# si220/Forest-SLAM

Measured on AMD Instinct MI355X. Metric: stereo frames/sec (extract+match+local-BA) at 600p, 1/8 MI355X; ATE RMSE, higher is better.
Workload: dtype mixed: u8/u16 integer (FAST, BRIEF, Hamming, SGM), f32 (ORB angle/Harris, back-projection), f64 (PnP, BA incl. its Schur GEMM on f64 MFMA); 1 GPU; stereo VO front end, configs[1]: 960x600, ORB nfeatures=1000, BF-Hamming xcheck (L+R), SGBM-3way 96 disp, back-projection, PnP-RANSAC, local BA K=10; width=960, height=600, nfeatures=1000, local_ba=window K=10 per frame, 10 LM iterations (fvo_ba_windows), parallelism=seq-per-gpu x1

## Files before the change

forest-slam_amd/csrc/ba.hip:

```cpp
#include <cfloat>
#include <type_traits>

#include "fvo_device.h"

namespace {

struct BaObs {
  int lm;
  short frame, oct;
  float u, v, ur;
};

struct BaCam {
  double fx, fy, cx, cy, b;
};

constexpr int kKMax = kBaMaxWindow;
constexpr int kBldL = 0, kBldO = kKMax, kBldTot = 2 * kKMax, kBldF = 2 * kKMax + 2, kBldInts = 3 * kKMax + 2;
constexpr int kBlock = 256;
constexpr int kLinParts = 12, kLinChunksPerPart = 8;
constexpr int kLinLPC64 = 64, kLinWavesDefault = 16;
static_assert(64 * kLinWavesDefault / (kLinLPC64 / 2) <= 64 && 64 * kLinWavesDefault / kLinLPC64 >= 16,
              "a landmark's lane group fits one wave and holds K observations");
constexpr int kLinWaves = kLinWavesDefault, kLinBlock = 64 * kLinWaves;
constexpr int kLinProd = kLinWaves / 2, kLinCons = kLinWaves - kLinProd;
constexpr int kLinMaxTiles = (36 + kLinCons - 1) / kLinCons;
constexpr int kLinTiles64 = (10 + kLinCons - 1) / kLinCons;
static_assert(kLinLPC64 / 2 <= 32 && (3 * (kLinLPC64 / 4)) % 4 == 0 && 3 * (kLinLPC64 / 2) / 4 <= 64,
              "half-chunk shape");
static_assert((64 * kLinProd) % (kLinLPC64 / 2) == 0, "producer lanes split evenly over a half chunk");
constexpr double kD2Mono = 5.991, kD2Stereo = 7.815, kMinZ = 0.01, kLam0 = 1e-3;

struct BaState {
  double T[kKMax][12], Tt[kKMax][12];
  double dp[6 * kKMax];
  double Hpp[kKMax][27];
  double lam, cost, cost0;
  int parity, fail, acc, active, L, O, n, s;
};

struct BaDims {
  int Lmax, Omax, K, cap, NR, LPC, NCH, NCU, NPART, LPU, NCUP;
  int64_t oSt, oX0, oX1, oL, oG, oLs, oObs, oFl, oGp, oCp, oNext, oHdr, oBld, win;
};

struct BaWin {
  BaState* st;
  double *X0, *X1, *Lf, *gl, *Gp, *cp;
  int *lstart, *flist, *next, *hdr, *bld;
  BaObs* obs;
};

__device__ __forceinline__ BaWin view(void* base, const BaDims& d, int w) {
  char* p = (char*)base + d.win * w;
  BaWin v;
  v.st = (BaState*)(p + d.oSt);
  v.X0 = (double*)(p + d.oX0);
  v.X1 = (double*)(p + d.oX1);
  v.Lf = (double*)(p + d.oL);
  v.gl = (double*)(p + d.oG);
  v.lstart = (int*)(p + d.oLs);
  v.obs = (BaObs*)(p + d.oObs);
  v.flist = (int*)(p + d.oFl);
  v.Gp = (double*)(p + d.oGp);
  v.cp = (double*)(p + d.oCp);
  v.next = (int*)(p + d.oNext);
  v.hdr = (int*)(p + d.oHdr);
  v.bld = (int*)(p + d.oBld);
  return v;
}

__global__ void k_ba_stereo(const int16_t* __restrict__ disp, const float* __restrict__ kp,
                            const int32_t* __restrict__ nkp, int W, int H, int cap, StereoCamF K,
                            float4* __restrict__ out) {
  const int b = blockIdx.y;
  const int i = blockIdx.x * blockDim.x + threadIdx.x;
  if (i >= cap) return;
  int n = nkp[b];
  float4 r = make_float4(0.f, 0.f, 0.f, 0.f);
  if (i < n) {
    const float* a = kp + ((int64_t)b * cap + i) * FVO_KP_STRIDE;
    const float x = a[0], y = a[1];
    int xi = min(max((int)x, 0), W - 1), yi = min(max((int)y, 0), H - 1);
    float d, X, Y;
    const float Z = stereo_depth(disp[((int64_t)b * H + yi) * W + xi], K.fxB, d);
    stereo_xy(x, y, Z, K, X, Y);
    if (Z > (float)0.1 && Z < 1000.f) r = make_float4(X, Y, Z, d);
  }
  out[(int64_t)b * cap + i] = r;
}

struct BaIn {
  const float* kp;
  const int32_t* nkp;
  const int32_t* matches;
  const int32_t* nmatch;
  const float4* stereo;
  const double* Trel;
  double isig2[FVO_MAX_LEVELS];
  int nlev;
};

__device__ __forceinline__ void mat_mul_T(const double* A, const double* B, double* C) {
  for (int i = 0; i < 3; ++i) {
    for (int j = 0; j < 3; ++j) C[3 * i + j] = A[3 * i] * B[j] + A[3 * i + 1] * B[3 + j] + A[3 * i + 2] * B[6 + j];
    C[9 + i] = A[3 * i] * B[9] + A[3 * i + 1] * B[10] + A[3 * i + 2] * B[11] + A[9 + i];
  }
}

__device__ __forceinline__ void pose_chain(const double* Trel, int s, int last, double* T, double (*out)[12]) {
  double U[12];
  for (int i = 0; i < 12; ++i) T[i] = (i < 9 && i % 4 == 0) ? 1.0 : 0.0;
  for (int k = 0; k <= last; ++k) {
    if (out)
      for (int i = 0; i < 12; ++i) out[k][i] = T[i];
    if (k < last) {
      const double* M = Trel + (int64_t)(s + k) * 16;
      const double A[12] = {M[0], M[1], M[2], M[4], M[5], M[6], M[8], M[9], M[10], M[3], M[7], M[11]};
// ... 292 lines not shown
      v.lstart[id] = o;
      const float* kq = in.kp + ((int64_t)b.f * dm.cap + q) * FVO_KP_STRIDE;
      const int oq = min(max((int)kq[5], 0), in.nlev - 1);
      v.obs[o++] = BaObs{id, (short)j, (short)oq, kq[0], kq[1], kq[0] - sp.w};
      float ku[kKMax - 1], kvv[kKMax - 1], ko[kKMax - 1];
#pragma unroll
      for (int kk = 0; kk < kKMax - 1; ++kk)
        if (kk < len - 1) {
          const float* kb = in.kp + ((int64_t)(b.f + 1 + kk) * dm.cap + bs[kk]) * FVO_KP_STRIDE;
          ku[kk] = kb[0];
          kvv[kk] = kb[1];
          ko[kk] = kb[5];
        }
#pragma unroll
      for (int kk = 0; kk < kKMax - 1; ++kk)
        if (kk < len - 1) {
          const int ob = min(max((int)ko[kk], 0), in.nlev - 1);
          v.obs[o++] = BaObs{id, (short)(j + 1 + kk), (short)ob, ku[kk], kvv[kk], __builtin_nanf("")};
        }
      for (int k = 0; k < len; ++k) atomicAdd(&s_fc[j + k], 1);
      ++okl;
      oko += len;
    }
    L0 += tp & 1023;
    O0 += tp >> 10;
    if (L0 >= dm.Lmax || O0 >= dm.Omax) break;
  }
  okl = block_sum<kBirthBlock>(okl, s_tmp);
  oko = block_sum<kBirthBlock>(oko, s_tmp);
  if (tid == 0) {
    atomicAdd(&v.bld[kBldTot], okl);
    atomicAdd(&v.bld[kBldTot + 1], oko);
  }
  if (tid < kKMax && s_fc[tid]) atomicAdd(&v.bld[kBldF + tid], s_fc[tid]);
}

__global__ __launch_bounds__(kBirthBlock) void k_ba_lists(BaIn in, void* ws, BaDims dm, int first_end,
                                                          int first_valid) {
  __shared__ int s_tmp[kBirthBlock / 64];
  const int w = blockIdx.x, k = blockIdx.y, tid = threadIdx.x;
  BaWin v = view(ws, dm, w);
  BaState* S = v.st;
  const int e = first_end + w, s = max(first_valid, e - dm.K + 1), n = e - s + 1;
  const bool live = n >= 3;
  const int L = live ? v.bld[kBldTot] : 0, O = live ? v.bld[kBldTot + 1] : 0;
  if (k == 0 && tid == 0) {
    S->L = L;
    S->O = O;
    S->n = n;
    S->s = s;
    S->active = L > 0;
    if (live) {
      v.lstart[L] = O;
      S->lam = kLam0;
      S->parity = 0;
      S->fail = 0;
      S->acc = 0;
      S->cost = 0.0;
      S->cost0 = 0.0;
      int acc = 0;
      for (int f = 0; f < n; ++f) {
        v.hdr[8 + f] = acc;
        acc += v.bld[kBldF + f];
      }
      v.hdr[8 + n] = acc;
      double T[12];
      pose_chain(in.Trel, s, n - 1, T, S->T);
    }
  }
  if (!live || k >= n || L == 0) return;
  int pos = 0;
  for (int f = 0; f < k; ++f) pos += v.bld[kBldF + f];
  for (int base = 0; base < L; base += kBirthBlock) {
    const int l = base + tid;
    int o0 = 0, jl = 0, len = 0;
    if (l < L) {
      o0 = v.lstart[l];
      len = (l + 1 < L ? v.lstart[l + 1] : O) - o0;
      jl = v.obs[o0].frame;
    }
    const bool sees = l < L && jl <= k && k < jl + len;
    int tot;
    const int rank = block_scan_excl<kBirthBlock>(sees ? 1 : 0, s_tmp, tot);
    if (sees) v.flist[pos + rank] = o0 + (k - jl);
    pos += tot;
  }
}

__device__ __forceinline__ const double* cur_X(const BaWin& v, const BaState* S) { return S->parity ? v.X1 : v.X0; }
__device__ __forceinline__ double* new_X(const BaWin& v, const BaState* S) { return S->parity ? v.X0 : v.X1; }

__global__ __launch_bounds__(kBlock) void k_ba_cost(BaIn in, void* ws, BaDims dm, BaCam cam, int reject) {
  __shared__ double s_red[kBlock / 64];
  const BaWin v = view(ws, dm, blockIdx.x);
  const BaState* S = v.st;
  if (!S->active) return;
  const int L = S->L, c = blockIdx.y;
  if (c * kBlock >= L) return;
  const double* X = cur_X(v, S);
  const int l = c * kBlock + threadIdx.x;
  double acc = 0;
  if (l < L) {
    for (int oi = v.lstart[l]; oi < v.lstart[l + 1]; ++oi) {
      BaObs o = v.obs[oi];
      if (reject && o.oct >= 0 && ba_outlier(S->T[o.frame], X + 3 * l, o, cam, in.isig2[o.oct])) {
        o.oct = -1;
        v.obs[oi].oct = -1;
      }
      double r[3], w, rho;
      ba_eval<false>(S->T[o.frame], X + 3 * l, o, cam, obs_is2(in, o), r, w, rho, nullptr, nullptr);
      acc += rho;
    }
  }
  const double t = block_sum<kBlock>(acc, s_red);
  if (threadIdx.x == 0) v.cp[c] = t;
}

__global__ void k_ba_setcost(void* ws, BaDims dm, int first) {
  const BaWin v = view(ws, dm, blockIdx.x);
  BaState* S = v.st;
  if (threadIdx.x != 0 || !S->active) return;
  const int nc = (S->L + kBlock - 1) / kBlock;
  double c = 0;
  for (int i = 0; i < nc; ++i) c += v.cp[i];
  S->cost = 0.5 * c;
  if (first) S->cost0 = 0.5 * c;
}

__global__ __launch_bounds__(kBlock) void k_ba_pp(BaIn in, void* ws, BaDims dm, BaCam cam) {
  const BaWin v = view(ws, dm, blockIdx.x);
  BaState* S = v.st;
  const int f = blockIdx.y + 1;
  if (!S->active || f >= S->n) return;
  const double* X = cur_X(v, S);
  const double* T = S->T[f];
  double h[27];
  for (int i = 0; i < 27; ++i) h[i] = 0;
  const int b0 = v.hdr[8 + f], b1 = v.hdr[8 + f + 1];
  for (int ii = b0 + threadIdx.x; ii < b1; ii += kBlock) {
    const int oi = v.flist[ii];
    const BaObs o = v.obs[oi];
    double r[3], w, rho, Jp[3][6];
    ba_eval<true, true, false>(T, X + 3 * o.lm, o, cam, obs_is2(in, o), r, w, rho, Jp, nullptr);
    int q = 0;
    for (int a = 0; a < 6; ++a) {
      for (int bb = a; bb < 6; ++bb) h[q++] += w * (Jp[0][a] * Jp[0][bb] + Jp[1][a] * Jp[1][bb] + Jp[2][a] * Jp[2][bb]);
      h[21 + a] += w * (Jp[0][a] * r[0] + Jp[1][a] * r[1] + Jp[2][a] * r[2]);
    }
  }
  __shared__ double s_part[kBlock / 64][27];
#pragma unroll
  for (int i = 0; i < 27; ++i) {
    const double wv = wave_sum(h[i]);
    if ((threadIdx.x & 63) == 0) s_part[threadIdx.x >> 6][i] = wv;
  }
  __syncthreads();
  if (threadIdx.x < 27) {
    double t = 0;
#pragma unroll
    for (int k = 0; k < kBlock / 64; ++k) t += s_part[k][threadIdx.x];
    S->Hpp[f][threadIdx.x] = t;
  }
}

__device__ __forceinline__ void lin_tile(int k, int ntu, int NT, int& I, int& J) {
  int idx = 0;
  for (int i = 0; i < ntu; ++i)
    for (int j = i; j < NT; ++j) {
      if (j >= ntu && j != NT - 1) continue;
      if (idx++ == k) { I = i; J = j; return; }
    }
  I = J = -1;
}

template <int CTRL>
__device__ __forceinline__ double dpp_f64(double v) {
  const uint64_t u = __builtin_bit_cast(uint64_t, v);
  const uint32_t lo = (uint32_t)__builtin_amdgcn_update_dpp(0, (int)(uint32_t)u, CTRL, 0xF, 0xF, false);
  const uint32_t hi = (uint32_t)__builtin_amdgcn_update_dpp(0, (int)(uint32_t)(u >> 32), CTRL, 0xF, 0xF, false);
  return __builtin_bit_cast(double, (uint64_t)hi << 32 | lo);
}
__device__ __forceinline__ double swz16_f64(double v) {
  const uint64_t u = __builtin_bit_cast(uint64_t, v);
  const uint32_t lo = (uint32_t)__builtin_amdgcn_ds_swizzle((int)(uint32_t)u, 0x401F);
  const uint32_t hi = (uint32_t)__builtin_amdgcn_ds_swizzle((int)(uint32_t)(u >> 32), 0x401F);
  return __builtin_bit_cast(double, (uint64_t)hi << 32 | lo);
}
template <int GL>
__device__ __forceinline__ double group_sum(double v) {
  static_assert(GL >= 2 && GL <= 32 && (GL & (GL - 1)) == 0, "group of 2..32 lanes");
  v += dpp_f64<0xB1>(v);
  if constexpr (GL >= 4) v += dpp_f64<0x4E>(v);
  if constexpr (GL >= 8) v += dpp_f64<0x141>(v);
  if constexpr (GL >= 16) v += dpp_f64<0x140>(v);
  if constexpr (GL >= 32) v += swz16_f64(v);
  return v;
}
template <int GL, int N>
__device__ __forceinline__ void group_sum_or(double (&v)[N], uint32_t& fm) {
#pragma unroll
  for (int q = 0; q < N; ++q) v[q] = group_sum<GL>(v[q]);
  fm |= (uint32_t)__builtin_amdgcn_update_dpp(0, (int)fm, 0xB1, 0xF, 0xF, false);
  if constexpr (GL >= 4) fm |= (uint32_t)__builtin_amdgcn_update_dpp(0, (int)fm, 0x4E, 0xF, 0xF, false);
  if constexpr (GL >= 8) fm |= (uint32_t)__builtin_amdgcn_update_dpp(0, (int)fm, 0x141, 0xF, 0xF, false);
  if constexpr (GL >= 16) fm |= (uint32_t)__builtin_amdgcn_update_dpp(0, (int)fm, 0x140, 0xF, 0xF, false);
  if constexpr (GL >= 32) fm |= (uint32_t)__builtin_amdgcn_ds_swizzle((int)fm, 0x401F);
}

template <int MAXT>
__global__ __launch_bounds__(kLinBlock) void k_ba_lin(BaIn in, void* ws, BaDims dm, BaCam cam) {
  extern __shared__ double sY[];
  __shared__ double sT[kKMax][12];
  __shared__ uint32_t s_tm[2][32];
  const BaWin v = view(ws, dm, blockIdx.x);
  const BaState* S = v.st;
  if (!S->active) return;
  const int L = S->L, part = blockIdx.y, LPC = dm.LPC, LPH = LPC / 2;
  if (part * LPC >= L) return;
  const int n = S->n;
  const int np = 6 * (n - 1);
  const int NR = dm.NR, NRP = NR + 2, rows = 3 * LPH;
  const int lane = threadIdx.x & 63, wid = threadIdx.x >> 6;
  const int NT = NR / 16, ntu = (np + 15) / 16;
  for (int i = threadIdx.x; i < n * 12; i += kLinBlock) sT[i / 12][i % 12] = S->T[i / 12][i % 12];
  const int nch = ((L + LPC - 1) / LPC - part + dm.NPART - 1) / dm.NPART, nh = 2 * nch;
  auto half_l0 = [&](int h) { return (part + (h >> 1) * dm.NPART) * LPC + (h & 1) * LPH; };
  __syncthreads();
  if (wid < kLinProd) {
    const double lam = S->lam;
    const double* X = cur_X(v, S);
    const int GL = kLinBlock / LPC, t = threadIdx.x / GL, j = threadIdx.x % GL;
    int ns0 = 0, ns1 = 0;
    BaObs onext{};
    double xn[3] = {0.0, 0.0, 0.0};
    auto fetch_start = [&](int h) {
      const int l = half_l0(h) + t;
      ns0 = ns1 = 0;
      if (h < nh && l < L) {
        ns0 = v.lstart[l];
        ns1 = v.lstart[l + 1];
        xn[0] = X[3 * l];
        xn[1] = X[3 * l + 1];
        xn[2] = X[3 * l + 2];
      }
    };
    auto fetch_obs = [&]() {
      if (j < ns1 - ns0) onext = v.obs[ns0 + j];
    };
    fetch_start(0);
    fetch_obs();
    for (int h = 0; h <= nh; ++h) {
      if (h < nh) {
        const BaObs o = onext;
        const int cnt = ns1 - ns0;
        const double xl[3] = {xn[0], xn[1], xn[2]};
        const int l = half_l0(h) + t;
        const bool live = l < L, has = live && j < cnt;
        fetch_start(h + 1);
        double hg[9] = {0, 0, 0, 0, 0, 0, 0, 0, 0};
        BaCoupling cpl{};
        const int f = has ? (int)o.frame : 0;
        if (has) {
          double r[3], rho, Jl[3][3];
          ba_eval_lw(sT[f], xl, o, cam, obs_is2(in, o), r, rho, Jl, cpl);
          const double w = cpl.w;
          int q = 0;
          for (int a2 = 0; a2 < 3; ++a2) {
            for (int b2 = a2; b2 < 3; ++b2) hg[q++] = w * (Jl[0][a2] * Jl[0][b2] + Jl[1][a2] * Jl[1][b2] + Jl[2][a2] * Jl[2][b2]);
            hg[6 + a2] = w * (Jl[0][a2] * r[0] + Jl[1][a2] * r[1] + Jl[2][a2] * r[2]);
          }
        }
        fetch_obs();
        uint32_t fm = has && f > 0 ? 1u << f : 0u;
        if (GL == 32) group_sum_or<32>(hg, fm);
        else if (GL == 16) group_sum_or<16>(hg, fm);
        else
          for (int m = GL >> 1; m >= 1; m >>= 1) {
#pragma unroll
            for (int q = 0; q < 9; ++q) hg[q] += __shfl_xor(hg[q], m, 64);
            fm |= (uint32_t)__shfl_xor((int)fm, m, 64);
          }
        const double* H = hg;
        const double a00 = H[0] + lam * H[0] + 1e-6, a11 = H[3] + lam * H[3] + 1e-6, a22 = H[5] + lam * H[5] + 1e-6;
// ... 88 lines not shown
          g = __builtin_ctzll(m);
          m &= m - 1;
        }
        double a1 = ya[4 * g * NRP], b1 = yb[4 * g * NRP];
        while (h1) {
          const bool h2 = m != 0;
          if (h2) {
            g = __builtin_ctzll(m);
            m &= m - 1;
          }
          const double a2 = ya[4 * g * NRP], b2 = yb[4 * g * NRP];
          acc[lt] = __builtin_amdgcn_mfma_f64_16x16x4f64(a0, b0, acc[lt], 0, 0, 0);
          a0 = a1, b0 = b1, a1 = a2, b1 = b2, h1 = h2;
        }
        acc[lt] = __builtin_amdgcn_mfma_f64_16x16x4f64(a0, b0, acc[lt], 0, 0, 0);
      }
    }
    __syncthreads();
  }
  double* Gc = v.Gp + (int64_t)part * NR * NR;
#pragma unroll
  for (int lt = 0; lt < MAXT; ++lt) {
    const int I = tI[lt], J = tJ[lt];
    if (I >= 0)
      for (int i = 0; i < 4; ++i) Gc[(16 * I + (lane >> 4) + 4 * i) * NR + 16 * J + (lane & 15)] = acc[lt][i];
  }
}

constexpr int kGsumParts = 2;
__global__ __launch_bounds__(256) void k_ba_gsum(void* ws, BaDims dm) {
  const BaWin v = view(ws, dm, blockIdx.x);
  const BaState* S = v.st;
  if (!S->active) return;
  const int nch0 = (S->L + dm.LPC - 1) / dm.LPC, nch = nch0 < dm.NPART ? nch0 : dm.NPART;
  const int64_t NN = (int64_t)dm.NR * dm.NR;
  const int64_t i2 = (int64_t)blockIdx.y * 256 + threadIdx.x;
  if (2 * i2 >= NN) return;
  typedef double d2 __attribute__((ext_vector_type(2)));
  d2* g = reinterpret_cast<d2*>(v.Gp) + i2;
  d2 part[kLinParts];
#pragma unroll
  for (int c = 0; c < kLinParts; ++c)
    if (c < nch) part[c] = g[c * (NN / 2)];
  d2 gs = {0.0, 0.0};
#pragma unroll
  for (int c = 0; c < kLinParts; ++c)
    if (c < nch) gs += part[c];
  g[0] = gs;
}

constexpr int kSolveBlock = 512, kSolveWaves = kSolveBlock / 64;
__host__ __device__ constexpr int ba_np16(int np) { return (np + 15) & ~15; }
__host__ __device__ constexpr int ba_sstride(int np16) { return np16 + 2; }
__global__ __launch_bounds__(kSolveBlock) void k_ba_solve(void* ws, BaDims dm) {
  extern __shared__ double sS[];
  __shared__ int s_fail;
  const BaWin v = view(ws, dm, blockIdx.x);
  BaState* S = v.st;
  if (!S->active) return;
  const int tid = threadIdx.x, lane = tid & 63, wid = tid >> 6;
  const int n = S->n, L = S->L, NR = dm.NR;
  const int np = 6 * (n - 1), NP = ba_np16(np), STR = ba_sstride(NP), NTl = NP / 16;
  const int nch0 = (L + dm.LPC - 1) / dm.LPC;
  const int nch = dm.NPART >= kGsumParts ? 1 : (nch0 < dm.NPART ? nch0 : dm.NPART);
  const double lam = S->lam;
  double* rhs = sS + NP * STR;
  double* rinv = rhs + NP;
  constexpr int LS = 17;
  double* linvT = rinv + NP;
  double* dcol = linvT + 17 * NP;
  if (tid == 0) s_fail = 0;
  double rhs_v = 0.0;
  if (tid < np) {
    double gs = 0.0;
    const double* gp = v.Gp + tid * NR + NR - 1;
    for (int c = 0; c < nch; ++c) gs += gp[(int64_t)c * NR * NR];
    rhs_v = -S->Hpp[tid / 6 + 1][21 + tid % 6] + gs;
  }
  const int pad = NP - np;
  for (int t = tid; t < pad * NP; t += kSolveBlock) {
    const int a = np + t / NP, b = t % NP;
    sS[a * STR + b] = a == b ? 1.0 : 0.0;
  }
  for (int t = tid; t < np * pad; t += kSolveBlock) sS[(t / pad) * STR + np + t % pad] = 0.0;
  typedef double d4 __attribute__((ext_vector_type(4)));
  const int nq = (np + 3) / 4;
  constexpr int kAsmIt = 8;
  static_assert(kAsmIt * kSolveBlock >= 6 * (kKMax - 1) * ((6 * (kKMax - 1) + 3) / 4),
                "every (row, column quad) of the largest reduced system is assembled");
  d4 gq[kAsmIt];
  double hq[kAsmIt][4];
#pragma unroll
  for (int k = 0; k < kAsmIt; ++k) {
    const int t = tid + k * kSolveBlock;
    const int a = t / nq, b0 = 4 * (t - a * nq);
    gq[k] = d4{0.0, 0.0, 0.0, 0.0};
#pragma unroll
    for (int u = 0; u < 4; ++u) hq[k][u] = 0.0;
    if (t >= np * nq || b0 + 3 < a) continue;
    const d4* gp = reinterpret_cast<const d4*>(v.Gp + a * NR + b0);
    d4 gs = {0.0, 0.0, 0.0, 0.0};
    for (int c = 0; c < nch; ++c) gs += gp[(int64_t)c * NR * NR / 4];
    gq[k] = gs;
    const int fa = a / 6 + 1, ia = a - 6 * (fa - 1);
#pragma unroll
    for (int u = 0; u < 4; ++u) {
      const int bb = b0 + u;
      if (bb < a || bb >= np || bb / 6 + 1 != fa) continue;
      const int j = bb - 6 * (fa - 1);
      hq[k][u] = S->Hpp[fa][ia * 6 - ia * (ia - 1) / 2 + (j - ia)];
    }
  }
#pragma unroll
  for (int k = 0; k < kAsmIt; ++k) {
    const int t = tid + k * kSolveBlock;
    const int a = t / nq, b0 = 4 * (t - a * nq);
    if (t >= np * nq || b0 + 3 < a) continue;
#pragma unroll
// ... 52 lines not shown
  auto panel_subst = [&](double (&x)[16], int c0) {
#pragma unroll
    for (int c = 0; c < 16; ++c) {
      x[c] *= rinv[c0 + c];
#pragma unroll
      for (int c2 = c + 1; c2 < 16; ++c2) x[c2] = fma(-x[c], sS[(c0 + c2) * STR + c0 + c], x[c2]);
    }
  };
  if (wid == 0) factor_diag(0);
  __syncthreads();
  for (int p = 0; p < NTl; ++p) {
    if (s_fail) break;
    const int c0 = 16 * p;
    const int nb = NP - c0 - 16;
    const bool unit = p == NTl - 1 && tid < 16;
    if (tid < nb || unit) {
      double* row = unit ? linvT + (p * 16 + tid) * LS : sS + (c0 + 16 + tid) * STR + c0;
      double x[16];
#pragma unroll
      for (int c = 0; c < 16; ++c) x[c] = unit ? (c == tid ? 1.0 : 0.0) : row[c];
      panel_subst(x, c0);
#pragma unroll
      for (int c = 0; c < 16; ++c) row[c] = x[c];
    }
    __syncthreads();
    const int m = NTl - p - 1;
    if (m > 0) {
      if (wid == 0) {
        tile_upd(c0, p + 1, p + 1);
        factor_diag(p + 1);
      } else {
        for (int t = wid; t < m * (m + 1) / 2; t += kSolveWaves - 1) {
          int I = p + 1, rem = t;
          while (rem >= I - p) {
            rem -= I - p;
            ++I;
          }
          tile_upd(c0, I, p + 1 + rem);
        }
        if (wid == kSolveWaves - 1 && lane < 16) {
          double x[16];
#pragma unroll
          for (int c = 0; c < 16; ++c) x[c] = c == lane ? 1.0 : 0.0;
          panel_subst(x, c0);
          double* row = linvT + (p * 16 + lane) * LS;
#pragma unroll
          for (int c = 0; c < 16; ++c) row[c] = x[c];
        }
      }
    }
    __syncthreads();
  }
  if (s_fail) {
    if (tid == 0) S->fail = 1;
    return;
  }
  if (wid == 0) {
    const int i = lane >> 2, q = lane & 3;
    auto quad_sum = [](double v) {
      v += dpp_f64<0xB1>(v);
      v += dpp_f64<0x4E>(v);
      return v;
    };
    auto lds_done = []() { asm volatile("s_waitcnt lgkmcnt(0)" ::: "memory"); };
    for (int p = 0; p < NTl; ++p) {
      const int c0 = 16 * p;
      const double* Lr = sS + (c0 + i) * STR;
      double a4[4] = {0.0, 0.0, 0.0, 0.0};
      for (int k0 = q; k0 < c0; k0 += 16)
#pragma unroll
        for (int u = 0; u < 4; ++u) a4[u] = fma(Lr[k0 + 4 * u], rhs[k0 + 4 * u], a4[u]);
      const double acc = quad_sum((a4[0] + a4[1]) + (a4[2] + a4[3]));
      const double r = rhs[c0 + i] - acc;
      lds_done();
      if (q == 0) rhs[c0 + i] = r;
      lds_done();
      const double* Li = linvT + p * 16 * LS;
      double y = 0.0;
#pragma unroll
      for (int u = 0; u < 4; ++u) y = fma(Li[(4 * q + u) * LS + i], rhs[c0 + 4 * q + u], y);
      y = quad_sum(y);
      lds_done();
      if (q == 0) rhs[c0 + i] = y;
      lds_done();
    }
    for (int p = NTl - 1; p >= 0; --p) {
      const int c0 = 16 * p;
      double a4[4] = {0.0, 0.0, 0.0, 0.0};
      for (int k0 = c0 + 16 + q; k0 < NP; k0 += 16)
#pragma unroll
        for (int u = 0; u < 4; ++u) a4[u] = fma(sS[(k0 + 4 * u) * STR + c0 + i], rhs[k0 + 4 * u], a4[u]);
      const double acc = quad_sum((a4[0] + a4[1]) + (a4[2] + a4[3]));
      const double t = rhs[c0 + i] - acc;
      lds_done();
      if (q == 0) rhs[c0 + i] = t;
      lds_done();
      const double* Li = linvT + (p * 16 + i) * LS;
      double x = 0.0;
#pragma unroll
      for (int u = 0; u < 4; ++u) x = fma(Li[4 * q + u], rhs[c0 + 4 * q + u], x);
      x = quad_sum(x);
      lds_done();
      if (q == 0) rhs[c0 + i] = x;
      lds_done();
    }
  }
  __syncthreads();
  for (int a = tid; a < 6 * n; a += kSolveBlock) S->dp[a] = a < 6 ? 0.0 : rhs[a - 6];
  if (tid < n) {
    const int f = tid;
    double* Tt = S->Tt[f];
    const double* T = S->T[f];
    if (f == 0) {
      for (int i = 0; i < 12; ++i) Tt[i] = T[i];
    } else {
      double Rw[9];
      const double* d = rhs + 6 * (f - 1);
      exp_so3(d, Rw);
      for (int i = 0; i < 3; ++i) {
        for (int j = 0; j < 3; ++j) Tt[3 * i + j] = Rw[3 * i] * T[j] + Rw[3 * i + 1] * T[3 + j] + Rw[3 * i + 2] * T[6 + j];
        Tt[9 + i] = Rw[3 * i] * T[9] + Rw[3 * i + 1] * T[10] + Rw[3 * i + 2] * T[11] + d[3 + i];
      }
    }
  }
}

constexpr int kUpdGluShort = 2, kUpdGluLong = 4;
template <int GLU>
__global__ __launch_bounds__(kBlock) void k_ba_upd(BaIn in, void* ws, BaDims dm, BaCam cam) {
  constexpr int LPU = kBlock / GLU;
  __shared__ double s_red[kBlock / 64];
  __shared__ double sT[kKMax][12], sTt[kKMax][12], sdp[kKMax][6];
  const BaWin v = view(ws, dm, blockIdx.x);
  const BaState* S = v.st;
  if (!S->active || S->fail) return;
  const int L = S->L, c = blockIdx.y;
  if (c * LPU >= L) return;
  const int n = S->n;
  for (int i = threadIdx.x; i < n * 12; i += kBlock) {
    sT[i / 12][i % 12] = S->T[i / 12][i % 12];
    sTt[i / 12][i % 12] = S->Tt[i / 12][i % 12];
  }
  for (int i = threadIdx.x; i < n * 6; i += kBlock) sdp[i / 6][i % 6] = S->dp[i];
  const double* X = cur_X(v, S);
  double* Xn = new_X(v, S);
  const int t = threadIdx.x / GLU, j = threadIdx.x % GLU, l = c * LPU + t;
  const bool live = l < L;
  int o0 = 0, o1 = 0;
  double Xc[3] = {0.0, 0.0, 0.0};
  if (live) {
    o0 = v.lstart[l];
    o1 = v.lstart[l + 1];
    Xc[0] = X[3 * l];
    Xc[1] = X[3 * l + 1];
    Xc[2] = X[3 * l + 2];
  }
  __syncthreads();
  double wd[3] = {0.0, 0.0, 0.0};
  for (int oi = o0 + j; oi < o1; oi += GLU) {
    const BaObs o = v.obs[oi];
    if (o.frame == 0) continue;
    double r[3], rho, Jl[3][3];
    BaCoupling cpl;
    ba_eval_lw(sT[o.frame], Xc, o, cam, obs_is2(in, o), r, rho, Jl, cpl);
    const double* dp = sdp[o.frame];
    double ow[3] = {0.0, 0.0, 0.0};
    for (int a = 0; a < 6; ++a) {
      double wr[3];
      ba_wrow(cpl, a, wr);
      for (int k = 0; k < 3; ++k) ow[k] += wr[k] * dp[a];
    }
    for (int k = 0; k < 3; ++k) wd[k] += ow[k];
  }
  for (int m = GLU >> 1; m >= 1; m >>= 1)
    for (int k = 0; k < 3; ++k) wd[k] += __shfl_xor(wd[k], m, 64);
  double rho = 0.0;
  if (live) {
    const double b0 = -v.gl[3 * l] - wd[0], b1 = -v.gl[3 * l + 1] - wd[1], b2 = -v.gl[3 * l + 2] - wd[2];
    const double* Lf = v.Lf + 6 * l;
    const double y0 = b0 / Lf[0], y1 = (b1 - Lf[1] * y0) / Lf[2], y2 = (b2 - Lf[3] * y0 - Lf[4] * y1) / Lf[5];
    const double x2 = y2 / Lf[5], x1 = (y1 - Lf[4] * x2) / Lf[2], x0 = (y0 - Lf[1] * x1 - Lf[3] * x2) / Lf[0];
    const double Xl[3] = {Xc[0] + x0, Xc[1] + x1, Xc[2] + x2};
    if (j == 0) {
      Xn[3 * l] = Xl[0];
      Xn[3 * l + 1] = Xl[1];
      Xn[3 * l + 2] = Xl[2];
    }
    for (int oi = o0 + j; oi < o1; oi += GLU) {
      const BaObs o = v.obs[oi];
      double r[3], w, ro;
      ba_eval<false>(sTt[o.frame], Xl, o, cam, obs_is2(in, o), r, w, ro, nullptr, nullptr);
      rho += ro;
    }
  }
  for (int m = GLU >> 1; m >= 1; m >>= 1) rho += __shfl_xor(rho, m, 64);
  const double tot = block_sum<kBlock>(j == 0 ? rho : 0.0, s_red);
  if (threadIdx.x == 0) v.cp[c] = tot;
}

__global__ __launch_bounds__(64) void k_ba_accept(void* ws, BaDims dm) {
  const BaWin v = view(ws, dm, blockIdx.x);
  BaState* S = v.st;
  if (!S->active) return;
  const int n = S->n;
  __shared__ int s_acc;
  __shared__ double s_sum;
  {
    const int nc = (S->L + dm.LPU - 1) / dm.LPU;
    double part = 0.0;
    if (!S->fail)
      for (int i = threadIdx.x; i < nc; i += 64) part += v.cp[i];
    part = wave_sum(part);
    if (threadIdx.x == 0) s_sum = 0.5 * part;
  }
  __syncthreads();
  if (threadIdx.x == 0) {
    s_acc = 0;
    if (S->fail) {
      S->lam = fmin(S->lam * 10.0, 1e7);
      S->fail = 0;
    } else {
      double c = s_sum;
      if (c < S->cost) {
        S->cost = c;
        S->lam = fmax(S->lam / 10.0, 1e-7);
        S->parity ^= 1;
        S->acc += 1;
        s_acc = 1;
      } else {
        S->lam = fmin(S->lam * 10.0, 1e7);
      }
    }
  }
  __syncthreads();
  if (s_acc)
    for (int i = threadIdx.x; i < n * 12; i += blockDim.x) S->T[i / 12][i % 12] = S->Tt[i / 12][i % 12];
}

__global__ void k_ba_final(const double* __restrict__ Trel, void* ws, BaDims dm, int first_end,
                           double* __restrict__ Tout_all, double* __restrict__ stats) {
  const int wi = blockIdx.x;
  const BaWin v = view(ws, dm, wi);
  const BaState* S = v.st;
  double* Tout = Tout_all + (int64_t)wi * 16;
  double* st = stats + (int64_t)wi * 6;
  if (threadIdx.x != 0) return;
  const int e = first_end + wi, n = S->n;
  if (!S->active) {
    for (int i = 0; i < 16; ++i) Tout[i] = Trel[(int64_t)(e - 1) * 16 + i];
    for (int i = 0; i < 6; ++i) st[i] = 0.0;
    st[4] = (double)n;
    return;
  }
  const double* A = S->T[n - 1];
  const double* B = S->T[n - 2];
  double Bi[12];
  for (int i = 0; i < 3; ++i)
    for (int j = 0; j < 3; ++j) Bi[3 * i + j] = B[3 * j + i];
  for (int i = 0; i < 3; ++i) Bi[9 + i] = -(Bi[3 * i] * B[9] + Bi[3 * i + 1] * B[10] + Bi[3 * i + 2] * B[11]);
  double C[12];
  mat_mul_T(A, Bi, C);
  for (int i = 0; i < 3; ++i) {
    for (int j = 0; j < 3; ++j) Tout[4 * i + j] = C[3 * i + j];
    Tout[4 * i + 3] = C[9 + i];
  }
  Tout[12] = Tout[13] = Tout[14] = 0.0;
  Tout[15] = 1.0;
  st[0] = S->cost0;
  st[1] = S->cost;
  st[2] = (double)S->L;
  st[3] = (double)S->O;
  st[4] = (double)n;
  st[5] = (double)S->acc;
}

__global__ void k_ba_export(void* ws, BaDims dm, int wi, double* __restrict__ xyz, int32_t* __restrict__ count) {
  const BaWin v = view(ws, dm, wi);
  const BaState* S = v.st;
  const int L = S->active ? S->L : 0;
  const double* X = cur_X(v, S);
  if (blockIdx.x == 0 && threadIdx.x == 0) *count = L;
  for (int i = blockIdx.x * blockDim.x + threadIdx.x; i < 3 * L; i += gridDim.x * blockDim.x) xyz[i] = X[i];
}

BaDims make_dims(const fvo_ctx* ctx) {
  const fvo_config& c = ctx->cfg;
  BaDims d{};
  d.Lmax = c.ba_max_landmarks;
  d.Omax = c.ba_max_obs;
  d.K = c.ba_window;
  d.cap = ctx->kp_cap;
  d.NR = 6 * (d.K - 1) < 63 ? 64 : 128;
  d.LPC = d.NR == 64 ? kLinLPC64 : kLinLPC64 / 2;
  d.NCH = (d.Lmax + d.LPC - 1) / d.LPC;
  d.NPART = d.NCH / kLinChunksPerPart;
  d.NPART = d.NPART < 1 ? 1 : d.NPART > kLinParts ? kLinParts : d.NPART;
  if (d.NPART > d.NCH) d.NPART = d.NCH;
  d.NCU = (d.Lmax + kBlock - 1) / kBlock;
  d.LPU = kBlock / (d.K <= 16 ? kUpdGluShort : kUpdGluLong);
  d.NCUP = (d.Lmax + d.LPU - 1) / d.LPU;
  int64_t o = 0;
  auto take = [&](int64_t bytes) {
    int64_t r = o;
    o += (bytes + 255) / 256 * 256;
    return r;
  };
  d.oSt = take((int64_t)sizeof(BaState));
  d.oX0 = take(8ll * 3 * d.Lmax);
  d.oX1 = take(8ll * 3 * d.Lmax);
  d.oL = take(8ll * 6 * d.Lmax);
  d.oG = take(8ll * 3 * d.Lmax);
  d.oLs = take(4ll * (d.Lmax + 1));
  d.oObs = take((int64_t)sizeof(BaObs) * d.Omax);
  d.oFl = take(4ll * d.Omax);
  d.oGp = take(8ll * d.NPART * d.NR * d.NR);
  d.oCp = take(8ll * (d.NCU > d.NCUP ? d.NCU : d.NCUP));
  d.oNext = take(4ll * kKMax * d.cap);
  d.oHdr = take(4ll * (8 + kKMax + 1));
  d.oBld = take(4ll * kBldInts);
  d.win = o;
  return d;
}

size_t build_shm(const BaDims& d) {
  const size_t maps = (size_t)2 * (d.K - 1) * d.cap + d.cap;
  return (d.cap < 0xFFFF && maps <= 156 * 1024) ? maps : (size_t)d.cap;
}
bool build_gmap(const BaDims& d) { return build_shm(d) == (size_t)d.cap; }

void ba_births_launch(const BaIn& in, void* ws, const BaDims& d, int nw, int fe, int first_valid, hipStream_t s) {
  const dim3 g(nw, d.K - 1), blk(kBirthBlock);
  const size_t shb = build_shm(d);
  if (build_gmap(d)) {
    hipLaunchKernelGGL(k_ba_maps, dim3(nw, d.K - 2), blk, 0, s, in, ws, d, fe, first_valid);
    hipLaunchKernelGGL(k_ba_births<true>, g, blk, shb, s, in, ws, d, fe, first_valid);
  } else {
    hipLaunchKernelGGL(k_ba_births<false>, g, blk, shb, s, in, ws, d, fe, first_valid);
  }
}
size_t lin_shm(const BaDims& d) { return (size_t)8 * 3 * d.LPC * (d.NR + 2); }
size_t solve_shm(int K) {
  const int np = 6 * (K - 1), NP = ba_np16(np);
  return (size_t)8 * (NP * ba_sstride(NP) + 2 * NP + 17 * NP + 16);
}

}

int ba_init(fvo_ctx* ctx) {
  const fvo_config& c = ctx->cfg;
  BaDims d = make_dims(ctx);
  ctx->ba_win_bytes = d.win;
  char* p = nullptr;
  int rc = fvo_alloc(ctx, &p, (size_t)d.win * c.max_batch);
  if (rc) return rc;
  ctx->ba_ws = p;
  FVO_HIP(ctx, hipStreamCreateWithFlags(&ctx->ba_s2, hipStreamNonBlocking));
  FVO_HIP(ctx, hipEventCreateWithFlags(&ctx->ba_fork, hipEventDisableTiming));
  FVO_HIP(ctx, hipEventCreateWithFlags(&ctx->ba_join, hipEventDisableTiming));
  if (build_shm(d) > 65536) {
    const bool g = build_gmap(d);
    FVO_HIP(ctx, hipFuncSetAttribute(g ? (const void*)k_ba_births<true> : (const void*)k_ba_births<false>,
                                     hipFuncAttributeMaxDynamicSharedMemorySize, (int)build_shm(d)));
    FVO_HIP(ctx, hipFuncSetAttribute(g ? (const void*)k_ba_emit<true> : (const void*)k_ba_emit<false>,
                                     hipFuncAttributeMaxDynamicSharedMemorySize, (int)build_shm(d)));
  }
  FVO_HIP(ctx, hipFuncSetAttribute((const void*)k_ba_lin<kLinTiles64>, hipFuncAttributeMaxDynamicSharedMemorySize,
                                   (int)lin_shm(d)));
  FVO_HIP(ctx, hipFuncSetAttribute((const void*)k_ba_lin<kLinMaxTiles>, hipFuncAttributeMaxDynamicSharedMemorySize,
                                   (int)lin_shm(d)));
  if (solve_shm(c.ba_window) > 65536)
    FVO_HIP(ctx, hipFuncSetAttribute((const void*)k_ba_solve, hipFuncAttributeMaxDynamicSharedMemorySize,
                                     (int)solve_shm(c.ba_window)));
  return 0;
}

int ba_stereo_run(fvo_ctx* ctx, const int16_t* disp, const float* kp, const int32_t* nkp, int batch, int cap,
                  const double* K, double baseline, float* stereo, hipStream_t s) {
  FVO_TIMED(ctx, KN_BA_STEREO, s,
            hipLaunchKernelGGL(k_ba_stereo, dim3((cap + 255) / 256, batch), dim3(256), 0, s, disp, kp, nkp,
                               ctx->cfg.width, ctx->cfg.height, cap, stereo_cam(K, baseline),
                               reinterpret_cast<float4*>(stereo)));
  FVO_LAUNCH_CHECK(ctx);
  return 0;
}

namespace {
void ba_windows_launch(fvo_ctx* ctx, const BaIn& in, const BaCam& cam, const BaDims& d, int w0, int nw, int first_end,
                       int first_valid, int iters, double* Tout, double* stats, hipStream_t s, bool births_done) {
  void* ws = static_cast<char*>(ctx->ba_ws) + (int64_t)d.win * w0;
  const int fe = first_end + w0;
  const size_t shb = build_shm(d);
  if (!births_done) ba_births_launch(in, ws, d, nw, fe, first_valid, s);
  if (build_gmap(d))
    hipLaunchKernelGGL(k_ba_emit<true>, dim3(nw, d.K - 1), dim3(kBirthBlock), shb, s, in, ws, d, fe, first_valid);
  else
    hipLaunchKernelGGL(k_ba_emit<false>, dim3(nw, d.K - 1), dim3(kBirthBlock), shb, s, in, ws, d, fe, first_valid);
  hipLaunchKernelGGL(k_ba_lists, dim3(nw, d.K), dim3(kBirthBlock), 0, s, in, ws, d, fe, first_valid);
  const dim3 gcu(nw, d.NCU), gch(nw, d.NPART), gfr(nw, d.K - 1);
  const size_t shl = lin_shm(d), shs = solve_shm(d.K);
  hipLaunchKernelGGL(k_ba_cost, gcu, dim3(kBlock), 0, s, in, ws, d, cam, 0);
  hipLaunchKernelGGL(k_ba_setcost, dim3(nw), dim3(64), 0, s, ws, d, 1);
  for (int it = 0; it < iters; ++it) {
    if (it == iters / 2 && iters >= 2) {
      hipLaunchKernelGGL(k_ba_cost, gcu, dim3(kBlock), 0, s, in, ws, d, cam, 1);
      hipLaunchKernelGGL(k_ba_setcost, dim3(nw), dim3(64), 0, s, ws, d, 0);
    }
    hipLaunchKernelGGL(k_ba_pp, gfr, dim3(kBlock), 0, s, in, ws, d, cam);
    if (d.NR == 64) hipLaunchKernelGGL(k_ba_lin<kLinTiles64>, gch, dim3(kLinBlock), shl, s, in, ws, d, cam);
    else hipLaunchKernelGGL(k_ba_lin<kLinMaxTiles>, gch, dim3(kLinBlock), shl, s, in, ws, d, cam);
    if (d.NPART >= kGsumParts)
      hipLaunchKernelGGL(k_ba_gsum, dim3(nw, (d.NR * d.NR / 2 + 255) / 256), dim3(256), 0, s, ws, d);
    hipLaunchKernelGGL(k_ba_solve, dim3(nw), dim3(kSolveBlock), shs, s, ws, d);
    if (d.K <= 16) hipLaunchKernelGGL(k_ba_upd<kUpdGluShort>, dim3(nw, d.NCUP), dim3(kBlock), 0, s, in, ws, d, cam);
    else hipLaunchKernelGGL(k_ba_upd<kUpdGluLong>, dim3(nw, d.NCUP), dim3(kBlock), 0, s, in, ws, d, cam);
    hipLaunchKernelGGL(k_ba_accept, dim3(nw), dim3(64), 0, s, ws, d);
  }
  hipLaunchKernelGGL(k_ba_final, dim3(nw), dim3(64), 0, s, in.Trel, ws, d, fe, Tout + 16 * (int64_t)w0,
                     stats + 6 * (int64_t)w0);
}
}

int ba_run(fvo_ctx* ctx, const float* kp, const int32_t* nkp, const int32_t* matches, const int32_t* nmatch,
           const float* stereo, const double* Trel, int nframes, int cap, int first_end, int nwin, int first_valid,
           const double* K, double baseline, const double* inv_sigma2, int nlev, int iters, double* Tout,
           double* stats, hipStream_t s) {
  const BaDims d = make_dims(ctx);
  BaIn in{kp, nkp, matches, nmatch, reinterpret_cast<const float4*>(stereo), Trel, {}, nlev};
  for (int i = 0; i < nlev; ++i) in.isig2[i] = inv_sigma2[i];
  const BaCam cam{K[0], K[4], K[2], K[5], baseline};
  const auto& pb = ctx->ba_births;
  const bool births_done = pb.valid && pb.matches == matches && pb.nmatch == nmatch && pb.stereo == stereo &&
                           pb.nframes == nframes && pb.first_end == first_end && pb.nwin == nwin &&
                           pb.first_valid == first_valid;
  ctx->ba_births.valid = false;
  const int nh = nwin >= 8 ? (nwin + 1) / 2 : nwin;
  const bool two = nh < nwin;
  if (two) {
    FVO_HIP(ctx, hipEventRecord(ctx->ba_fork, s));
    FVO_HIP(ctx, hipStreamWaitEvent(ctx->ba_s2, ctx->ba_fork, 0));
  }
  FVO_TIMED(ctx, KN_BA_SOLVE, s, {
    ba_windows_launch(ctx, in, cam, d, 0, nh, first_end, first_valid, iters, Tout, stats, s, births_done);
    if (two)
      ba_windows_launch(ctx, in, cam, d, nh, nwin - nh, first_end, first_valid, iters, Tout, stats, ctx->ba_s2,
                        births_done);
    if (two) {
      (void)hipEventRecord(ctx->ba_join, ctx->ba_s2);
      (void)hipStreamWaitEvent(s, ctx->ba_join, 0);
    }
  });
  FVO_LAUNCH_CHECK(ctx);
  return 0;
}

int ba_births_run(fvo_ctx* ctx, const int32_t* matches, const int32_t* nmatch, const float* stereo, int nframes,
                  int cap, int first_end, int nwin, int first_valid, hipStream_t s) {
  const BaDims d = make_dims(ctx);
  BaIn in{nullptr, nullptr, matches, nmatch, reinterpret_cast<const float4*>(stereo), nullptr, {}, 1};
  ba_births_launch(in, ctx->ba_ws, d, nwin, first_end, first_valid, s);
  FVO_LAUNCH_CHECK(ctx);
  auto& pb = ctx->ba_births;
  pb.valid = true;
  pb.matches = matches;
  pb.nmatch = nmatch;
  pb.stereo = stereo;
  pb.nframes = nframes;
  pb.first_end = first_end;
  pb.nwin = nwin;
  pb.first_valid = first_valid;
  return 0;
}
// ... 8 lines not shown
```

Measured before the change: 6065 frames/s.

## Fold LM accept and set-cost kernels into consumers via double-buffered LM state

Removes the separate k_ba_setcost and k_ba_accept launches from the local bundle-adjustment loop. The Levenberg-Marquardt bookkeeping (cost reduction, lambda update, parity flip) is now recomputed redundantly at the start of the next consuming kernel (pp, cost, final) and written into a ping-pong BaLm slot. Poses become double-buffered by parity, so accepting a step no longer requires copying T from Tt. This drops one or two small serial launches per iteration. The cost is redundant reductions in every block of the consuming kernels and more intricate state indexing.

```diff
diff --git a/forest-slam_amd/csrc/ba.hip b/forest-slam_amd/csrc/ba.hip
--- a/forest-slam_amd/csrc/ba.hip
+++ b/forest-slam_amd/csrc/ba.hip
@@ -31,22 +31,28 @@
 static_assert((64 * kLinProd) % (kLinLPC64 / 2) == 0, "producer lanes split evenly over a half chunk");
 constexpr double kD2Mono = 5.991, kD2Stereo = 7.815, kMinZ = 0.01, kLam0 = 1e-3;
 
+struct BaLm {
+  double lam, cost;
+  int parity, fail, acc, pad;
+};
 struct BaState {
-  double T[kKMax][12], Tt[kKMax][12];
+  double P[2][kKMax][12];
   double dp[6 * kKMax];
   double Hpp[kKMax][27];
-  double lam, cost, cost0;
-  int parity, fail, acc, active, L, O, n, s;
+  BaLm lm[2];
+  double cost0;
+  int parity;
+  int active, L, O, n, s;
 };
 
 struct BaDims {
   int Lmax, Omax, K, cap, NR, LPC, NCH, NCU, NPART, LPU, NCUP;
-  int64_t oSt, oX0, oX1, oL, oG, oLs, oObs, oFl, oGp, oCp, oNext, oHdr, oBld, win;
+  int64_t oSt, oX0, oX1, oL, oG, oLs, oObs, oFl, oGp, oCp, oCu, oNext, oHdr, oBld, win;
 };
 
 struct BaWin {
   BaState* st;
-  double *X0, *X1, *Lf, *gl, *Gp, *cp;
+  double *X0, *X1, *Lf, *gl, *Gp, *cp, *cu;
   int *lstart, *flist, *next, *hdr, *bld;
   BaObs* obs;
 };
@@ -64,6 +70,7 @@
   v.flist = (int*)(p + d.oFl);
   v.Gp = (double*)(p + d.oGp);
   v.cp = (double*)(p + d.oCp);
+  v.cu = (double*)(p + d.oCu);
   v.next = (int*)(p + d.oNext);
   v.hdr = (int*)(p + d.oHdr);
   v.bld = (int*)(p + d.oBld);
@@ -462,12 +469,9 @@
     S->active = L > 0;
     if (live) {
       v.lstart[L] = O;
-      S->lam = kLam0;
+      S->lm[0] = BaLm{kLam0, 0.0, 0, 0, 0, 0};
+      S->cost0 = 0.0;
       S->parity = 0;
-      S->fail = 0;
-      S->acc = 0;
-      S->cost = 0.0;
-      S->cost0 = 0.0;
       int acc = 0;
       for (int f = 0; f < n; ++f) {
         v.hdr[8 + f] = acc;
@@ -475,7 +479,7 @@
       }
       v.hdr[8 + n] = acc;
       double T[12];
-      pose_chain(in.Trel, s, n - 1, T, S->T);
+      pose_chain(in.Trel, s, n - 1, T, S->P[0]);
     }
   }
   if (!live || k >= n || L == 0) return;
@@ -497,28 +501,67 @@
   }
 }
 
-__device__ __forceinline__ const double* cur_X(const BaWin& v, const BaState* S) { return S->parity ? v.X1 : v.X0; }
-__device__ __forceinline__ double* new_X(const BaWin& v, const BaState* S) { return S->parity ? v.X0 : v.X1; }
-
-__global__ __launch_bounds__(kBlock) void k_ba_cost(BaIn in, void* ws, BaDims dm, BaCam cam, int reject) {
+__device__ __forceinline__ const double* cur_X(const BaWin& v, int parity) { return parity ? v.X1 : v.X0; }
+__device__ __forceinline__ double* new_X(const BaWin& v, int parity) { return parity ? v.X0 : v.X1; }
+
+enum { kLmKeep = 0, kLmAccept = 1, kLmCost = 2, kLmCostFirst = 3 };
+__device__ __forceinline__ BaLm lm_next(const BaWin& v, const BaState* S, const BaDims& dm, int g, int mode) {
+  BaLm m = S->lm[g];
+  if (mode == kLmAccept) {
+    if (m.fail) {
+      m.lam = fmin(m.lam * 10.0, 1e7);
+      m.fail = 0;
+    } else {
+      const int nc = (S->L + dm.LPU - 1) / dm.LPU;
+      double part = 0.0;
+      for (int i = threadIdx.x & 63; i < nc; i += 64) part += v.cu[i];
+      const double c = 0.5 * wave_sum(part);
+      if (c < m.cost) {
+        m.cost = c;
+        m.lam = fmax(m.lam / 10.0, 1e-7);
+        m.parity ^= 1;
+        m.acc += 1;
+      } else {
+        m.lam = fmin(m.lam * 10.0, 1e7);
+      }
+    }
+  } else if (mode != kLmKeep) {
+    const int nc = (S->L + kBlock - 1) / kBlock;
+    double c = 0;
+    for (int i = 0; i < nc; ++i) c += v.cp[i];
+    m.cost = 0.5 * c;
+  }
+  return m;
+}
+__device__ __forceinline__ void lm_store(BaState* S, const BaLm& m, int g, int mode) {
+  if (mode == kLmKeep || blockIdx.y != 0 || threadIdx.x != 0) return;
+  S->lm[g ^ 1] = m;
+  if (mode == kLmCostFirst) S->cost0 = m.cost;
+}
+
+__global__ __launch_bounds__(kBlock) void k_ba_cost(BaIn in, void* ws, BaDims dm, BaCam cam, int reject, int g,
+                                                    int mode) {
   __shared__ double s_red[kBlock / 64];
   const BaWin v = view(ws, dm, blockIdx.x);
-  const BaState* S = v.st;
+  BaState* S = v.st;
   if (!S->active) return;
+  const BaLm lm = lm_next(v, S, dm, g, mode);
+  lm_store(S, lm, g, mode);
   const int L = S->L, c = blockIdx.y;
   if (c * kBlock >= L) return;
-  const double* X = cur_X(v, S);
+  const double* X = cur_X(v, lm.parity);
+  const double(*T)[12] = S->P[lm.parity];
   const int l = c * kBlock + threadIdx.x;
   double acc = 0;
   if (l < L) {
     for (int oi = v.lstart[l]; oi < v.lstart[l + 1]; ++oi) {
       BaObs o = v.obs[oi];
-      if (reject && o.oct >= 0 && ba_outlier(S->T[o.frame], X + 3 * l, o, cam, in.isig2[o.oct])) {
+      if (reject && o.oct >= 0 && ba_outlier(T[o.frame], X + 3 * l, o, cam, in.isig2[o.oct])) {
         o.oct = -1;
         v.obs[oi].oct = -1;
       }
       double r[3], w, rho;
-      ba_eval<false>(S->T[o.frame], X + 3 * l, o, cam, obs_is2(in, o), r, w, rho, nullptr, nullptr);
+      ba_eval<false>(T[o.frame], X + 3 * l, o, cam, obs_is2(in, o), r, w, rho, nullptr, nullptr);
       acc += rho;
     }
   }
@@ -526,24 +569,15 @@
   if (threadIdx.x == 0) v.cp[c] = t;
 }
 
-__global__ void k_ba_setcost(void* ws, BaDims dm, int first) {
-  const BaWin v = view(ws, dm, blockIdx.x);
-  BaState* S = v.st;
-  if (threadIdx.x != 0 || !S->active) return;
-  const int nc = (S->L + kBlock - 1) / kBlock;
-  double c = 0;
-  for (int i = 0; i < nc; ++i) c += v.cp[i];
-  S->cost = 0.5 * c;
-  if (first) S->cost0 = 0.5 * c;
-}
-
-__global__ __launch_bounds__(kBlock) void k_ba_pp(BaIn in, void* ws, BaDims dm, BaCam cam) {
+__global__ __launch_bounds__(kBlock) void k_ba_pp(BaIn in, void* ws, BaDims dm, BaCam cam, int g, int mode) {
   const BaWin v = view(ws, dm, blockIdx.x);
   BaState* S = v.st;
   const int f = blockIdx.y + 1;
   if (!S->active || f >= S->n) return;
-  const double* X = cur_X(v, S);
-  const double* T = S->T[f];
+  const BaLm lm = lm_next(v, S, dm, g, mode);
+  lm_store(S, lm, g, mode);
+  const double* X = cur_X(v, lm.parity);
+  const double* T = S->P[lm.parity][f];
   double h[27];
   for (int i = 0; i < 27; ++i) h[i] = 0;
   const int b0 = v.hdr[8 + f], b1 = v.hdr[8 + f + 1];
@@ -618,7 +652,7 @@
 }
 
 template <int MAXT>
-__global__ __launch_bounds__(kLinBlock) void k_ba_lin(BaIn in, void* ws, BaDims dm, BaCam cam) {
+__global__ __launch_bounds__(kLinBlock) void k_ba_lin(BaIn in, void* ws, BaDims dm, BaCam cam, int g) {
   extern __shared__ double sY[];
   __shared__ double sT[kKMax][12];
   __shared__ uint32_t s_tm[2][32];
@@ -632,13 +666,14 @@
   const int NR = dm.NR, NRP = NR + 2, rows = 3 * LPH;
   const int lane = threadIdx.x & 63, wid = threadIdx.x >> 6;
   const int NT = NR / 16, ntu = (np + 15) / 16;
-  for (int i = threadIdx.x; i < n * 12; i += kLinBlock) sT[i / 12][i % 12] = S->T[i / 12][i % 12];
+  const int parity = S->lm[g].parity;
+  for (int i = threadIdx.x; i < n * 12; i += kLinBlock) sT[i / 12][i % 12] = S->P[parity][i / 12][i % 12];
   const int nch = ((L + LPC - 1) / LPC - part + dm.NPART - 1) / dm.NPART, nh = 2 * nch;
   auto half_l0 = [&](int h) { return (part + (h >> 1) * dm.NPART) * LPC + (h & 1) * LPH; };
   __syncthreads();
   if (wid < kLinProd) {
-    const double lam = S->lam;
-    const double* X = cur_X(v, S);
+    const double lam = S->lm[g].lam;
+    const double* X = cur_X(v, parity);
     const int GL = kLinBlock / LPC, t = threadIdx.x / GL, j = threadIdx.x % GL;
     int ns0 = 0, ns1 = 0;
     BaObs onext{};
@@ -833,7 +868,7 @@
 constexpr int kSolveBlock = 512, kSolveWaves = kSolveBlock / 64;
 __host__ __device__ constexpr int ba_np16(int np) { return (np + 15) & ~15; }
 __host__ __device__ constexpr int ba_sstride(int np16) { return np16 + 2; }
-__global__ __launch_bounds__(kSolveBlock) void k_ba_solve(void* ws, BaDims dm) {
+__global__ __launch_bounds__(kSolveBlock) void k_ba_solve(void* ws, BaDims dm, int g) {
   extern __shared__ double sS[];
   __shared__ int s_fail;
   const BaWin v = view(ws, dm, blockIdx.x);
@@ -844,7 +879,8 @@
   const int np = 6 * (n - 1), NP = ba_np16(np), STR = ba_sstride(NP), NTl = NP / 16;
   const int nch0 = (L + dm.LPC - 1) / dm.LPC;
   const int nch = dm.NPART >= kGsumParts ? 1 : (nch0 < dm.NPART ? nch0 : dm.NPART);
-  const double lam = S->lam;
+  const double lam = S->lm[g].lam;
+  const int parity = S->lm[g].parity;
   double* rhs = sS + NP * STR;
   double* rinv = rhs + NP;
   constexpr int LS = 17;
@@ -1003,7 +1039,7 @@
     __syncthreads();
   }
   if (s_fail) {
-    if (tid == 0) S->fail = 1;
+    if (tid == 0) S->lm[g].fail = 1;
     return;
   }
   if (wid == 0) {
@@ -1060,8 +1096,8 @@
   for (int a = tid; a < 6 * n; a += kSolveBlock) S->dp[a] = a < 6 ? 0.0 : rhs[a - 6];
   if (tid < n) {
     const int f = tid;
-    double* Tt = S->Tt[f];
-    const double* T = S->T[f];
+    double* Tt = S->P[parity ^ 1][f];
+    const double* T = S->P[parity][f];
     if (f == 0) {
       for (int i = 0; i < 12; ++i) Tt[i] = T[i];
     } else {
@@ -1078,23 +1114,23 @@
 
 constexpr int kUpdGluShort = 2, kUpdGluLong = 4;
 template <int GLU>
-__global__ __launch_bounds__(kBlock) void k_ba_upd(BaIn in, void* ws, BaDims dm, BaCam cam) {
+__global__ __launch_bounds__(kBlock) void k_ba_upd(BaIn in, void* ws, BaDims dm, BaCam cam, int g) {
   constexpr int LPU = kBlock / GLU;
   __shared__ double s_red[kBlock / 64];
   __shared__ double sT[kKMax][12], sTt[kKMax][12], sdp[kKMax][6];
   const BaWin v = view(ws, dm, blockIdx.x);
   const BaState* S = v.st;
-  if (!S->active || S->fail) return;
+  if (!S->active || S->lm[g].fail) return;
   const int L = S->L, c = blockIdx.y;
   if (c * LPU >= L) return;
-  const int n = S->n;
+  const int n = S->n, parity = S->lm[g].parity;
   for (int i = threadIdx.x; i < n * 12; i += kBlock) {
-    sT[i / 12][i % 12] = S->T[i / 12][i % 12];
-    sTt[i / 12][i % 12] = S->Tt[i / 12][i % 12];
+    sT[i / 12][i % 12] = S->P[parity][i / 12][i % 12];
+    sTt[i / 12][i % 12] = S->P[parity ^ 1][i / 12][i % 12];
   }
   for (int i = threadIdx.x; i < n * 6; i += kBlock) sdp[i / 6][i % 6] = S->dp[i];
-  const double* X = cur_X(v, S);
-  double* Xn = new_X(v, S);
+  const double* X = cur_X(v, parity);
+  double* Xn = new_X(v, parity);
   const int t = threadIdx.x / GLU, j = threadIdx.x % GLU, l = c * LPU + t;
   const bool live = l < L;
   int o0 = 0, o1 = 0;
@@ -1146,55 +1182,19 @@
   }
   for (int m = GLU >> 1; m >= 1; m >>= 1) rho += __shfl_xor(rho, m, 64);
   const double tot = block_sum<kBlock>(j == 0 ? rho : 0.0, s_red);
-  if (threadIdx.x == 0) v.cp[c] = tot;
-}
-
-__global__ __launch_bounds__(64) void k_ba_accept(void* ws, BaDims dm) {
-  const BaWin v = view(ws, dm, blockIdx.x);
-  BaState* S = v.st;
-  if (!S->active) return;
-  const int n = S->n;
-  __shared__ int s_acc;
-  __shared__ double s_sum;
-  {
-    const int nc = (S->L + dm.LPU - 1) / dm.LPU;
-    double part = 0.0;
-    if (!S->fail)
-      for (int i = threadIdx.x; i < nc; i += 64) part += v.cp[i];
-    part = wave_sum(part);
-    if (threadIdx.x == 0) s_sum = 0.5 * part;
-  }
-  __syncthreads();
-  if (threadIdx.x == 0) {
-    s_acc = 0;
-    if (S->fail) {
-      S->lam = fmin(S->lam * 10.0, 1e7);
-      S->fail = 0;
-    } else {
-      double c = s_sum;
-      if (c < S->cost) {
-        S->cost = c;
-        S->lam = fmax(S->lam / 10.0, 1e-7);
-        S->parity ^= 1;
-        S->acc += 1;
-        s_acc = 1;
-      } else {
-        S->lam = fmin(S->lam * 10.0, 1e7);
-      }
-    }
-  }
-  __syncthreads();
-  if (s_acc)
-    for (int i = threadIdx.x; i < n * 12; i += blockDim.x) S->T[i / 12][i % 12] = S->Tt[i / 12][i % 12];
-}
-
-__global__ void k_ba_final(const double* __restrict__ Trel, void* ws, BaDims dm, int first_end,
-                           double* __restrict__ Tout_all, double* __restrict__ stats) {
+  if (threadIdx.x == 0) v.cu[c] = tot;
+}
+
+__global__ __launch_bounds__(64) void k_ba_final(const double* __restrict__ Trel, void* ws, BaDims dm, int first_end,
+                                                 double* __restrict__ Tout_all, double* __restrict__ stats, int g,
+                                                 int mode) {
   const int wi = blockIdx.x;
   const BaWin v = view(ws, dm, wi);
-  const BaState* S = v.st;
+  BaState* S = v.st;
   double* Tout = Tout_all + (int64_t)wi * 16;
   double* st = stats + (int64_t)wi * 6;
+  BaLm lm{};
+  if (S->active) lm = lm_next(v, S, dm, g, mode);
   if (threadIdx.x != 0) return;
   const int e = first_end + wi, n = S->n;
   if (!S->active) {
@@ -1203,8 +1203,9 @@
     st[4] = (double)n;
     return;
   }
-  const double* A = S->T[n - 1];
-  const double* B = S->T[n - 2];
+  S->parity = lm.parity;
+  const double* A = S->P[lm.parity][n - 1];
+  const double* B = S->P[lm.parity][n - 2];
   double Bi[12];
   for (int i = 0; i < 3; ++i)
     for (int j = 0; j < 3; ++j) Bi[3 * i + j] = B[3 * j + i];
@@ -1217,19 +1218,19 @@
   }
   Tout[12] = Tout[13] = Tout[14] = 0.0;
   Tout[15] = 1.0;
-  st[0] = S->cost0;
-  st[1] = S->cost;
+  st[0] = mode == kLmCostFirst ? lm.cost : S->cost0;
+  st[1] = lm.cost;
   st[2] = (double)S->L;
   st[3] = (double)S->O;
   st[4] = (double)n;
-  st[5] = (double)S->acc;
+  st[5] = (double)lm.acc;
 }
 
 __global__ void k_ba_export(void* ws, BaDims dm, int wi, double* __restrict__ xyz, int32_t* __restrict__ count) {
   const BaWin v = view(ws, dm, wi);
   const BaState* S = v.st;
   const int L = S->active ? S->L : 0;
-  const double* X = cur_X(v, S);
+  const double* X = cur_X(v, S->parity);
   if (blockIdx.x == 0 && threadIdx.x == 0) *count = L;
   for (int i = blockIdx.x * blockDim.x + threadIdx.x; i < 3 * L; i += gridDim.x * blockDim.x) xyz[i] = X[i];
 }
@@ -1265,7 +1266,8 @@
   d.oObs = take((int64_t)sizeof(BaObs) * d.Omax);
   d.oFl = take(4ll * d.Omax);
   d.oGp = take(8ll * d.NPART * d.NR * d.NR);
-  d.oCp = take(8ll * (d.NCU > d.NCUP ? d.NCU : d.NCUP));
+  d.oCp = take(8ll * d.NCU);
+  d.oCu = take(8ll * d.NCUP);
   d.oNext = take(4ll * kKMax * d.cap);
   d.oHdr = take(4ll * (8 + kKMax + 1));
   d.oBld = take(4ll * kBldInts);
@@ -1349,25 +1351,27 @@
   hipLaunchKernelGGL(k_ba_lists, dim3(nw, d.K), dim3(kBirthBlock), 0, s, in, ws, d, fe, first_valid);
   const dim3 gcu(nw, d.NCU), gch(nw, d.NPART), gfr(nw, d.K - 1);
   const size_t shl = lin_shm(d), shs = solve_shm(d.K);
-  hipLaunchKernelGGL(k_ba_cost, gcu, dim3(kBlock), 0, s, in, ws, d, cam, 0);
-  hipLaunchKernelGGL(k_ba_setcost, dim3(nw), dim3(64), 0, s, ws, d, 1);
+  int g = 0, open = kLmCostFirst;
+  hipLaunchKernelGGL(k_ba_cost, gcu, dim3(kBlock), 0, s, in, ws, d, cam, 0, g, (int)kLmKeep);
   for (int it = 0; it < iters; ++it) {
     if (it == iters / 2 && iters >= 2) {
-      hipLaunchKernelGGL(k_ba_cost, gcu, dim3(kBlock), 0, s, in, ws, d, cam, 1);
-      hipLaunchKernelGGL(k_ba_setcost, dim3(nw), dim3(64), 0, s, ws, d, 0);
-    }
-    hipLaunchKernelGGL(k_ba_pp, gfr, dim3(kBlock), 0, s, in, ws, d, cam);
-    if (d.NR == 64) hipLaunchKernelGGL(k_ba_lin<kLinTiles64>, gch, dim3(kLinBlock), shl, s, in, ws, d, cam);
-    else hipLaunchKernelGGL(k_ba_lin<kLinMaxTiles>, gch, dim3(kLinBlock), shl, s, in, ws, d, cam);
+      hipLaunchKernelGGL(k_ba_cost, gcu, dim3(kBlock), 0, s, in, ws, d, cam, 1, g, open);
+      g ^= 1;
+      open = kLmCost;
+    }
+    hipLaunchKernelGGL(k_ba_pp, gfr, dim3(kBlock), 0, s, in, ws, d, cam, g, open);
+    g ^= 1;
+    open = kLmAccept;
+    if (d.NR == 64) hipLaunchKernelGGL(k_ba_lin<kLinTiles64>, gch, dim3(kLinBlock), shl, s, in, ws, d, cam, g);
+    else hipLaunchKernelGGL(k_ba_lin<kLinMaxTiles>, gch, dim3(kLinBlock), shl, s, in, ws, d, cam, g);
     if (d.NPART >= kGsumParts)
       hipLaunchKernelGGL(k_ba_gsum, dim3(nw, (d.NR * d.NR / 2 + 255) / 256), dim3(256), 0, s, ws, d);
-    hipLaunchKernelGGL(k_ba_solve, dim3(nw), dim3(kSolveBlock), shs, s, ws, d);
-    if (d.K <= 16) hipLaunchKernelGGL(k_ba_upd<kUpdGluShort>, dim3(nw, d.NCUP), dim3(kBlock), 0, s, in, ws, d, cam);
-    else hipLaunchKernelGGL(k_ba_upd<kUpdGluLong>, dim3(nw, d.NCUP), dim3(kBlock), 0, s, in, ws, d, cam);
-    hipLaunchKernelGGL(k_ba_accept, dim3(nw), dim3(64), 0, s, ws, d);
+    hipLaunchKernelGGL(k_ba_solve, dim3(nw), dim3(kSolveBlock), shs, s, ws, d, g);
+    if (d.K <= 16) hipLaunchKernelGGL(k_ba_upd<kUpdGluShort>, dim3(nw, d.NCUP), dim3(kBlock), 0, s, in, ws, d, cam, g);
+    else hipLaunchKernelGGL(k_ba_upd<kUpdGluLong>, dim3(nw, d.NCUP), dim3(kBlock), 0, s, in, ws, d, cam, g);
   }
   hipLaunchKernelGGL(k_ba_final, dim3(nw), dim3(64), 0, s, in.Trel, ws, d, fe, Tout + 16 * (int64_t)w0,
-                     stats + 6 * (int64_t)w0);
+                     stats + 6 * (int64_t)w0, g, open);
 }
 }
 
```

Result: no change. 6077 frames/s, median of 2 (+0.2%).
